# ylsung/vl-merging

Measured on AMD Instinct MI355X. Metric: VL samples/sec (fwd+bwd) base_vl 384^2 at 1/2/4/8 GPUs; merge GB/s vs HBM peak, higher is better.
Workload: dtype bf16

## Files before the change

### include/vlm_hip.h

```cpp
#ifndef VLM_HIP_H
#define VLM_HIP_H
#include <stddef.h>
#include <stdint.h>

#ifdef __cplusplus
extern "C" {
#endif

#define VLM_OK 0
#define VLM_ERR_ARG (-1)
#define VLM_ERR_LAUNCH (-2)
#define VLM_ERR_WORKSPACE (-3)
#define VLM_ERR_UNSUPPORTED (-4)

#define VLM_ABI_VERSION 10
int vlm_abi_version(void);
int vlm_device_cus(void);
int vlm_set_cu_budget(int cus);
int vlm_debug_occupy(int workgroups, int threads, int lds_bytes, int microseconds, void* stream);

#define VLM_MERGE_LERP 0
#define VLM_MERGE_TASKVEC 1
#define VLM_MERGE_MEAN 2
#define VLM_MERGE_MAX_SRC 4
// ... 70 lines not shown

int vlm_gemm_bf16(int ta, int tb, int M, int N, int K, const void* A, int lda, const void* B, int ldb, void* C,
                  int ldc, int c_is_f32, const vlm_epilogue_t* epi, void* stream);
#define VLM_GEMM_MAX_GROUPS 4
typedef struct {
  int32_t row0, rows;
  const void* B;
  int32_t ldb;
  int32_t reserved;
  const float* bias;
  float* col_sum;
  float* col_sum_ws;
} vlm_gemm_group_t;
int vlm_gemm_bf16_grouped(int n_groups, const vlm_gemm_group_t* groups, int N, int K, const void* A, int lda, void* C,
                          int ldc, int c_is_f32, const vlm_epilogue_t* epi, void* stream);
typedef struct {
  int32_t row0, rows;
  float* C;
  int32_t accumulate;
  int32_t reserved;
} vlm_wgrad_group_t;
int vlm_gemm_wgrad_grouped(int n_groups, const vlm_wgrad_group_t* groups, int M, int N, const void* A, int lda,
                           const void* B, int ldb, int ldc, float* splitk_ws, uint64_t splitk_ws_bytes, void* stream);
int vlm_gemm_set_big_tile_mode(int mode);

int vlm_layernorm_fwd(const float* x, int ldx, int M, int D, const float* gamma, const float* beta, float eps,
                      void* y, int ldy, int y_is_f32, float* stats, void* stream);
#define VLM_ROW_WS_BYTES(D) ((size_t)1536 * 2 * (size_t)(D) * sizeof(float))
int vlm_layernorm_bwd(const void* dy, int lddy, int dy_is_f32, const float* x, int ldx, const float* stats,
                      const float* gamma, int M, int D, const float* dres, int lddres, float* dx, int lddx,
                      float* dgamma, float* dbeta, float* workspace, size_t workspace_bytes, int* deferred_blocks,
                      void* stream);
typedef struct {
  const void* y;
  int32_t ldy;
  const float* gamma;
  const float* row_scale;
  void* dy;
  int32_t lddy;
  float* dgamma;
  float* dbias;
  float* workspace;
  size_t workspace_bytes;
} vlm_layerscale_t;
int vlm_layernorm_bwd_scale(const void* dy, int lddy, int dy_is_f32, const float* x, int ldx, const float* stats,
                            const float* gamma, int M, int D, const float* dres, int lddres, float* dx, int lddx,
// ... 156 lines not shown
```

### vl-merging_amd/_lib.py

```python
import ctypes
import os

_HERE = os.path.dirname(os.path.abspath(__file__))
LIB_PATH = os.environ.get("VLM_LIB_PATH") or os.path.join(_HERE, "lib", "libvlm_hip.so")
_lib = None

c_void_p = ctypes.c_void_p
c_int = ctypes.c_int
c_float = ctypes.c_float
c_size_t = ctypes.c_size_t
c_u64 = ctypes.c_uint64

MERGE_LERP, MERGE_TASKVEC, MERGE_MEAN = 0, 1, 2
MERGE_MAX_SRC = 4


class MergeJob(ctypes.Structure):
    _fields_ = [
        ("dst", c_void_p),
        ("base", c_void_p),
        ("src", c_void_p * MERGE_MAX_SRC),
        ("ratio", c_float * MERGE_MAX_SRC),
        ("n_src", ctypes.c_int32),
        ("mode", ctypes.c_int32),
# ... 30 lines not shown
                ("row_step", ctypes.c_int32), ("count", ctypes.c_int32)]


class Epilogue(ctypes.Structure):
    _fields_ = [
        ("bias", c_void_p), ("col_scale", c_void_p), ("row_scale", c_void_p), ("residual", c_void_p),
        ("ld_res", ctypes.c_int64), ("aux", c_void_p), ("ld_aux", ctypes.c_int64), ("act", ctypes.c_int32),
        ("alpha", c_float), ("accumulate", ctypes.c_int32), ("reserved", ctypes.c_int32), ("col_sum", c_void_p),
        ("col_sum_ws", c_void_p), ("splitk_ws", c_void_p), ("splitk_ws_bytes", ctypes.c_uint64),
    ]


GEMM_MAX_GROUPS = 4


class GemmGroup(ctypes.Structure):
    _fields_ = [("row0", ctypes.c_int32), ("rows", ctypes.c_int32), ("B", c_void_p), ("ldb", ctypes.c_int32),
                ("reserved", ctypes.c_int32), ("bias", c_void_p), ("col_sum", c_void_p), ("col_sum_ws", c_void_p)]


class WgradGroup(ctypes.Structure):
    _fields_ = [("row0", ctypes.c_int32), ("rows", ctypes.c_int32), ("C", c_void_p), ("accumulate", ctypes.c_int32),
                ("reserved", ctypes.c_int32)]


class FoldJob(ctypes.Structure):
    _fields_ = [("partials", c_void_p), ("nblocks", ctypes.c_int32), ("D", ctypes.c_int32), ("out0", c_void_p),
                ("out1", c_void_p)]


class LayerScale(ctypes.Structure):
    _fields_ = [("y", c_void_p), ("ldy", ctypes.c_int32), ("gamma", c_void_p), ("row_scale", c_void_p), ("dy", c_void_p),
                ("lddy", ctypes.c_int32), ("dgamma", c_void_p), ("dbias", c_void_p), ("workspace", c_void_p),
                ("workspace_bytes", c_size_t)]


class AttnColsum(ctypes.Structure):
    _fields_ = [("dq", c_void_p * 2), ("dv", c_void_p * 2)]


ACT_NONE, ACT_GELU, ACT_GELU_BWD, ACT_GELU_DERIV, ACT_MUL_AUX = 0, 1, 2, 3, 4
ATTN_JOINT, ATTN_SEPARATE = 0, 1


class AttnDesc(ctypes.Structure):
    _fields_ = [
# ... 22 lines not shown


_ERR = {-1: "VLM_ERR_ARG", -2: "VLM_ERR_LAUNCH", -3: "VLM_ERR_WORKSPACE", -4: "VLM_ERR_UNSUPPORTED"}

SIGNATURES = {
    "vlm_abi_version": (c_int, []),
    "vlm_device_cus": (c_int, []),
    "vlm_set_cu_budget": (c_int, [c_int]),
    "vlm_debug_occupy": (c_int, [c_int, c_int, c_int, c_int, c_void_p]),
    "vlm_layerscale_fold": (c_int, [ctypes.POINTER(LayerScaleJob), c_int, c_void_p]),
    "vlm_layerscale_finish": (c_int, [ctypes.POINTER(LayerScaleJob), c_int, c_void_p]),
    "vlm_merge_plan_bytes": (c_size_t, [c_int, c_u64]),
    "vlm_merge_plan_upload": (c_int, [ctypes.POINTER(MergeJob), c_int, c_void_p, c_size_t, c_void_p]),
    "vlm_merge_run": (c_int, [c_void_p, c_void_p]),
    "vlm_ties_plan_bytes": (c_size_t, [c_int, c_u64]),
    "vlm_ties_plan_upload": (c_int, [ctypes.POINTER(TiesJob), c_int, c_void_p, c_size_t, c_void_p]),
    "vlm_ties_run": (c_int, [c_void_p, c_void_p]),
    "vlm_gemm_bf16": (c_int, [c_int, c_int, c_int, c_int, c_int, c_void_p, c_int, c_void_p, c_int, c_void_p, c_int,
                              c_int, ctypes.POINTER(Epilogue), c_void_p]),
    "vlm_gemm_bf16_grouped": (c_int, [c_int, ctypes.POINTER(GemmGroup), c_int, c_int, c_void_p, c_int, c_void_p, c_int, c_int,
                                      ctypes.POINTER(Epilogue), c_void_p]),
    "vlm_gemm_wgrad_grouped": (c_int, [c_int, ctypes.POINTER(WgradGroup), c_int, c_int, c_void_p, c_int, c_void_p, c_int, c_int,
                                       c_void_p, c_u64, c_void_p]),
    "vlm_attention_fwd": (c_int, [ctypes.POINTER(AttnDesc), c_void_p, c_int, c_void_p, c_void_p]),
    "vlm_attention_bwd_ws_floats": (c_size_t, [ctypes.POINTER(AttnDesc), c_int]),
    "vlm_attention_bwd": (c_int, [ctypes.POINTER(AttnDesc), c_void_p, c_int, c_void_p, c_int, c_void_p, c_void_p, c_size_t,
                                  c_void_p, c_int, c_void_p, c_void_p, c_void_p]),
    "vlm_layernorm_fwd": (c_int, [c_void_p, c_int, c_int, c_int, c_void_p, c_void_p, c_float, c_void_p, c_int, c_int,
                                  c_void_p, c_void_p]),
    "vlm_layernorm_bwd": (c_int, [c_void_p, c_int, c_int, c_void_p, c_int, c_void_p, c_void_p, c_int, c_int, c_void_p,
                                  c_int, c_void_p, c_int, c_void_p, c_void_p, c_void_p, c_size_t,
                                  ctypes.POINTER(c_int), c_void_p]),
    "vlm_layernorm_bwd_scale": (c_int, [c_void_p, c_int, c_int, c_void_p, c_int, c_void_p, c_void_p, c_int, c_int, c_void_p,
                                        c_int, c_void_p, c_int, c_void_p, c_void_p, c_void_p, c_size_t,
                                        ctypes.POINTER(LayerScale), ctypes.POINTER(c_int), c_void_p]),
    "vlm_layerscale_bwd": (c_int, [c_void_p, c_int, c_void_p, c_int, c_void_p, c_void_p, c_int, c_int, c_void_p, c_int,
                                   c_void_p, c_void_p, c_void_p, c_size_t, ctypes.POINTER(c_int), c_void_p]),
    "vlm_colreduce_batch": (c_int, [ctypes.POINTER(FoldJob), c_int, c_void_p]),
    "vlm_gemm_set_big_tile_mode": (c_int, [c_int]),
    "vlm_colsum_bf16": (c_int, [c_void_p, c_int, c_int, c_int, c_void_p, c_void_p]),
    "vlm_adamw_step": (c_int, [c_void_p, c_void_p, c_void_p, c_void_p, c_void_p, c_u64, c_float, c_float, c_float,
                               c_float, c_float, c_float, c_float, c_int, c_void_p]),
    "vlm_accumulate_f32_f64": (c_int, [c_void_p, c_void_p, c_u64, c_void_p]),
    "vlm_gram_f64": (c_int, [c_void_p, c_int, c_int, c_int, c_int, c_void_p, c_void_p]),
    "vlm_gemm_f64": (c_int, [c_int, c_int, c_int, c_int, c_int, ctypes.c_double, c_void_p, c_int, c_int, c_void_p, c_int,
                             ctypes.c_double, c_void_p, c_int, c_void_p]),
# ... 85 lines not shown
```

### vl-merging_amd/csrc/gemm.hip

```cpp
#include "vlm_common.h"
#include "vlm_diag.h"
#include <atomic>

#define GEMM_BM 128
#define GEMM_BN 128
#define GEMM_BK 64
#define GEMM_THREADS 256
#define GEMM_TILE_BYTES (GEMM_BM * GEMM_BK * 2)

typedef __attribute__((address_space(3))) s16x4 lds_s16x4;

__device__ __forceinline__ float gelu_cdf(float x, float& ez2) {
  const float t = __builtin_amdgcn_rcpf(fmaf(0.3275911f * 0.70710678118654752440f, fabsf(x), 1.0f));
  ez2 = __builtin_amdgcn_exp2f((x * x) * (-0.5f * 1.4426950408889634f));
  float poly = fmaf(t, 0.5f * 1.061405429f, 0.5f * -1.453152027f);
  poly = fmaf(t, poly, 0.5f * 1.421413741f);
  poly = fmaf(t, poly, 0.5f * -0.284496736f);
  poly = fmaf(t, poly, 0.5f * 0.254829592f);
  const float e = fmaf(-(poly * t), ez2, 0.5f);
  return 0.5f + copysignf(e, x);
}
__device__ __forceinline__ float gelu_erf(float x) {
  float ez2;
  return x * gelu_cdf(x, ez2);
}
// ... 885 lines not shown
#define BIG_TAIL_STEPS()                                                               \
  BIG_STEP(kt + 0, 0, 1, 1, fa0, fb0, fa1, fb1, ra0, rb0, sA0, sB0, sA1, sB1)          \
  BIG_STEP(kt + 1, 0, 1, 1, fa1, fb1, fa0, fb0, ra1, rb1, sA1, sB1, sA0, sB0)          \
  BIG_STEP(kt + 2, 0, 0, 1, fa0, fb0, fa1, fb1, ra0, rb0, sA0, sB0, sA1, sB1)          \
  BIG_STEP(kt + 3, 0, 0, 0, fa1, fb1, fa0, fb0, ra1, rb1, sA1, sB1, sA0, sB0)
  if constexpr (DEEP) {
    BIG_TAIL_STEPS()
    GEMM_STAMP(2)
    big_epilogue_t<OUT_F32, RES, AUX> ep(p, wl, mw0, nw0, lane);
    float* ws_row = (p.epi.col_sum_ws && mw0 + 128 <= (uint32_t)p.M) ? p.epi.col_sum_ws + ((size_t)(tm_ws * 2 + wm) * 2) * p.N : nullptr;
    BIG_EPILOGUE_LOOP_DEEP(AHEAD)
    ep.finish(lane, ws_row);
  } else {
    EPIL_SETUP()
    BIG_TAIL_STEPS()
    GEMM_STAMP(2)
    float* ws_row = (p.epi.col_sum_ws && mw0 + 128 <= (uint32_t)p.M) ? p.epi.col_sum_ws + ((size_t)(tm_ws * 2 + wm) * 2) * p.N : nullptr;
    BIG_EPILOGUE_LOOP()
    ep.finish(lane, ws_row);
  }
  GEMM_STAMP_END()
}

template <bool GROUPED = false>
__global__ __launch_bounds__(GEMM_THREADS, 1) void vlm_gemm_bigT_kernel(const gemm_params_t p) {
  __shared__ __attribute__((aligned(1024))) unsigned char sA0[BIG_OP_BYTES], sA1[BIG_OP_BYTES], sB0[BIG_OP_BYTES], sB1[BIG_OP_BYTES];
  __shared__ __attribute__((aligned(16))) unsigned char epl[4 * EPIL_WAVE_BYTES];
  const int tid = threadIdx.x;
  const int lane = tid & 63;
  const int wave = __builtin_amdgcn_readfirstlane(tid >> 6);
  const int wm = wave >> 1, wn = wave & 1;
  const uint32_t ntile = p.tiles_m * p.tiles_n;
  const uint32_t q8 = gridDim.x >> 3, r8 = gridDim.x & 7, xcd = blockIdx.x & 7;
  uint32_t item = (xcd < r8 ? xcd * (q8 + 1) : r8 * (q8 + 1) + (xcd - r8) * q8) + (blockIdx.x >> 3);
  uint32_t k_base = 0, k_end = (uint32_t)p.K, slice0 = 0;
  int nk = p.ksteps_per_split;
  if constexpr (GROUPED) {
    int g = 0;
#pragma unroll
    for (int i = 1; i < VLM_GEMM_MAX_GROUPS; ++i)
      if (i < p.n_groups && item >= (uint32_t)p.grpT[i].item0) g = i;
    const gemmT_group_t G = p.grpT[g];
    item -= (uint32_t)G.item0;
    k_base = (uint32_t)G.row0;
    k_end = (uint32_t)G.row_end;
    nk = G.kps;
    slice0 = (uint32_t)G.slice0;
  }
  const uint32_t split = item / ntile, tile = item - split * ntile;
  const uint32_t tm = tile / p.tiles_n, tn = tile - tm * p.tiles_n;
  const uint32_t m0 = tm * BIG_BM, n0 = tn * BIG_BN;
  const uint32_t k_first = k_base + split * (uint32_t)nk * BIG_BK;
  const __amdgpu_buffer_rsrc_t ra =
      __builtin_amdgcn_make_buffer_rsrc(const_cast<void*>(p.A), 0, (int)((uint64_t)k_end * p.lda * 2), 0x00020000);
  const __amdgpu_buffer_rsrc_t rb =
      __builtin_amdgcn_make_buffer_rsrc(const_cast<void*>(p.B), 0, (int)((uint64_t)k_end * p.ldb * 2), 0x00020000);

  uint32_t offa[4], offb[4], wr_off[4];
#pragma unroll
  for (int u = 0; u < 4; ++u) {
    const uint32_t row = 2 * (wave + 4 * u) + (lane >> 5), c16 = lane & 31;
    offa[u] = ((k_first + row) * (uint32_t)p.lda + m0 + c16 * 8) * 2;
    offb[u] = ((k_first + row) * (uint32_t)p.ldb + n0 + c16 * 8) * 2;
    wr_off[u] = row * 512 + (((c16 >> 1) ^ ((row & 3) | (((row >> 3) & 1) << 2))) << 5) + (c16 & 1) * 16;
  }
  uint32_t rda[8], rdb[8];
  {
    const uint32_t g = lane >> 4, q = (lane & 15) >> 2, pp = lane & 3, sw = q | ((g & 1) << 2);
#pragma unroll
    for (int i = 0; i < 8; ++i) {
      rda[i] = (8 * g + q) * 512 + wm * 256 + ((i ^ sw) << 5) + 8 * pp;
      rdb[i] = (8 * g + q) * 512 + wn * 256 + ((i ^ sw) << 5) + 8 * pp;
    }
  }
  f32x4 acc00[4][4], acc01[4][4], acc10[4][4], acc11[4][4];
#pragma unroll
  for (int i = 0; i < 4; ++i)
#pragma unroll
    for (int j = 0; j < 4; ++j) {
      acc00[i][j] = (f32x4){0.f, 0.f, 0.f, 0.f};
      acc01[i][j] = (f32x4){0.f, 0.f, 0.f, 0.f};
      acc10[i][j] = (f32x4){0.f, 0.f, 0.f, 0.f};
      acc11[i][j] = (f32x4){0.f, 0.f, 0.f, 0.f};
    }
  const uint32_t stepa = BIG_BK * (uint32_t)p.lda * 2, stepb = BIG_BK * (uint32_t)p.ldb * 2;
  bf16x8 fa0[8], fb0[8], fa1[8], fb1[8];
  u32x4 ra0[4], rb0[4], ra1[4], rb1[4];
#define BIGT_TR(PTR) __builtin_amdgcn_ds_read_tr16_b64_v4i16((lds_s16x4*)(PTR))
#define BIGT_READ(FA, FB, SA, SB)                                                                    \
  _Pragma("unroll") for (int i = 0; i < 8; ++i) {                                                    \
    const s16x4 al = BIGT_TR((SA) + rda[i]), ah = BIGT_TR((SA) + rda[i] + 4 * 512);                  \
    const s16x4 bl = BIGT_TR((SB) + rdb[i]), bh = BIGT_TR((SB) + rdb[i] + 4 * 512);                  \
    FA[i] = __builtin_bit_cast(bf16x8, (s16x8){al[0], al[1], al[2], al[3], ah[0], ah[1], ah[2], ah[3]}); \
    FB[i] = __builtin_bit_cast(bf16x8, (s16x8){bl[0], bl[1], bl[2], bl[3], bh[0], bh[1], bh[2], bh[3]}); \
  }
#define BIGT_GLOAD(RA_, RB_, S)                                                                      \
  _Pragma("unroll") for (int u = 0; u < 4; ++u) {                                                    \
    RA_[u] = __builtin_amdgcn_raw_buffer_load_b128(ra, offa[u], (S) * stepa, 0);                     \
    RB_[u] = __builtin_amdgcn_raw_buffer_load_b128(rb, offb[u], (S) * stepb, 0);                     \
  }
#define BIGT_LWRITE(RA_, RB_, SA, SB)                                                                \
  _Pragma("unroll") for (int u = 0; u < 4; ++u) {                                                    \
    *reinterpret_cast<u32x4*>((SA) + wr_off[u]) = RA_[u];                                            \
    *reinterpret_cast<u32x4*>((SB) + wr_off[u]) = RB_[u];                                            \
  }
#define BIGT_STEP(K, GL, WR, RD, FCA, FCB, FNA, FNB, RSA, RSB, BUFA_W, BUFB_W, BUFA_R, BUFB_R)      \
  {                                                                                      \
    if (RD) {                                                                            \
// ... 17 lines not shown
    }                                                                                    \
    __builtin_amdgcn_sched_barrier(0);                                                   \
  }
  BIGT_GLOAD(ra0, rb0, 0)
  BIGT_GLOAD(ra1, rb1, 1)
  BIGT_LWRITE(ra0, rb0, sA0, sB0)
  BIGT_GLOAD(ra0, rb0, 2)
  BIGT_LWRITE(ra1, rb1, sA1, sB1)
  BIGT_GLOAD(ra1, rb1, 3)
  asm volatile("s_waitcnt lgkmcnt(0)" ::: "memory");
  __builtin_amdgcn_s_barrier();
  BIGT_READ(fa0, fb0, sA0, sB0)
  int kt = 0;
  for (; kt < nk - 4; kt += 2) {
    BIGT_STEP(kt + 0, 1, 1, 1, fa0, fb0, fa1, fb1, ra0, rb0, sA0, sB0, sA1, sB1)
    BIGT_STEP(kt + 1, 1, 1, 1, fa1, fb1, fa0, fb0, ra1, rb1, sA1, sB1, sA0, sB0)
  }
  BIGT_STEP(kt + 0, 0, 1, 1, fa0, fb0, fa1, fb1, ra0, rb0, sA0, sB0, sA1, sB1)
  BIGT_STEP(kt + 1, 0, 1, 1, fa1, fb1, fa0, fb0, ra1, rb1, sA1, sB1, sA0, sB0)
  BIGT_STEP(kt + 2, 0, 0, 1, fa0, fb0, fa1, fb1, ra0, rb0, sA0, sB0, sA1, sB1)
  BIGT_STEP(kt + 3, 0, 0, 0, fa1, fb1, fa0, fb0, ra1, rb1, sA1, sB1, sA0, sB0)

  gemm_params_t pl = p;
  pl.C = reinterpret_cast<float*>(p.C) + (size_t)(slice0 + split) * p.M * p.N;
  pl.ldc = p.N;
  const uint32_t mw0 = m0 + wm * 128, nw0 = n0 + wn * 128;
  unsigned char* const wl = epl + wave * EPIL_WAVE_BYTES;
  big_epilogue_t<true, false, 0, 128, 0, true> ep(pl, wl, mw0, nw0, lane);
  epil_in_t inA, inB;
  ep.load_inputs(inA, 0);
  BIG_EPILOGUE_LOOP()
}

__global__ __launch_bounds__(256) void splitk_reduce_kernel(const float* __restrict__ ws, int splits, int M, int N, float* __restrict__ C,
                                                            int ldc, int accumulate) {
  const size_t i = (size_t)blockIdx.x * 256 + threadIdx.x, per = (size_t)M * N / 4;
  if (i >= per) return;
  const size_t e = i * 4, m = e / N, n = e - m * N;
  f32x4 t = accumulate ? *reinterpret_cast<const f32x4*>(C + m * ldc + n) : (f32x4){0.f, 0.f, 0.f, 0.f};
  for (int s = 0; s < splits; ++s) t += *reinterpret_cast<const f32x4*>(ws + (size_t)s * M * N + e);
  *reinterpret_cast<f32x4*>(C + m * ldc + n) = t;
}

struct splitk_groups_t {
  float* C[VLM_GEMM_MAX_GROUPS];
  int slice0[VLM_GEMM_MAX_GROUPS], splits[VLM_GEMM_MAX_GROUPS], accumulate[VLM_GEMM_MAX_GROUPS];
};
__global__ __launch_bounds__(256) void splitk_reduce_grouped_kernel(const float* __restrict__ ws, const splitk_groups_t g, int M, int N, int ldc) {
  const size_t i = (size_t)blockIdx.x * 256 + threadIdx.x, per = (size_t)M * N / 4;
  if (i >= per) return;
  const int gi = blockIdx.y;
  float* const C = g.C[gi];
  const size_t e = i * 4, m = e / N, n = e - m * N;
  f32x4 t = g.accumulate[gi] ? *reinterpret_cast<const f32x4*>(C + m * ldc + n) : (f32x4){0.f, 0.f, 0.f, 0.f};
// ... 296 lines not shown
      VLM_CHECK_LAUNCH();
      const size_t per = (size_t)M * N / 4;
      hipLaunchKernelGGL(splitk_reduce_grouped_kernel, dim3((unsigned)((per + 255) / 256), p.n_groups), dim3(256), 0, s,
                         reinterpret_cast<const float*>(splitk_ws), rg, M, N, ldc);
      VLM_CHECK_LAUNCH();
      return VLM_OK;
    }
  }
  for (int g = 0; g < n_groups; ++g) {
    const vlm_wgrad_group_t& G = groups[g];
    if (G.rows == 0) continue;
    vlm_epilogue_t e{};
    e.alpha = 1.0f;
    e.accumulate = G.accumulate;
    e.splitk_ws = splitk_ws;
    e.splitk_ws_bytes = splitk_ws_bytes;
    const size_t r0 = (size_t)G.row0;
    const int rc = vlm_gemm_bf16(1, 1, M, N, G.rows, reinterpret_cast<const unsigned char*>(A) + r0 * lda * 2, lda,
                                 reinterpret_cast<const unsigned char*>(B) + r0 * ldb * 2, ldb, G.C, ldc, 1, &e, stream);
    if (rc) return rc;
  }
  return VLM_OK;
}
```

### vl-merging_amd/engine.py

```python
import itertools
import math
import os
import weakref
from typing import List, Optional

import torch

from . import _lib as L
from . import ops

BF16, F32 = torch.bfloat16, torch.float32
ALIGN = 64


def _touch_hook(p):
    p._vlm_flat.touched.add(p._vlm_name)


def touch(*params):
    for p in params:
        if p is not None:
            f = getattr(p, "_vlm_flat", None)
            if f is not None:
                f.touched.add(p._vlm_name)
# ... 208 lines not shown
        return False


def wT16(p):
    s = getattr(p, "_vlm_bf16_t", None)
    if s is None:
        raise L.VlmError("weight has no transposed bf16 shadow: call model.setup_engine() on a CUDA model first")
    return s


def _gemm_rows(a, groups, out, *, act=L.ACT_NONE, aux=None, col_scale=None, row_scale=None, residual=None, col_sum_fold=None):
    if len(groups) > 1:
        return ops.gemm_grouped(a, groups, out, act=act, aux=aux, col_scale=col_scale, row_scale=row_scale,
                                residual=residual, col_sum_fold=col_sum_fold)
    (r0, r1, w, bias, col_sum), = groups

    def rows(t):
        return t[r0:r1] if t is not None else None

    return ops.gemm(a[r0:r1], w, out[r0:r1], bias=bias, act=act, aux=rows(aux), col_scale=col_scale,
                    row_scale=rows(row_scale), residual=rows(residual), col_sum=col_sum, col_sum_fold=col_sum_fold)


def _wgrad_rows(dy, x, groups):
    if len(groups) > 1:
        return ops.gemm_wgrad_grouped(dy, x, groups)
    (r0, r1, dw), = groups
    return ops.gemm(dy[r0:r1], x[r0:r1], dw, ta=True, tb=True, accumulate=True)


def w16(p):
    s = getattr(p, "_vlm_bf16", None)
    if s is None:
        raise L.VlmError("parameter has no bf16 shadow: call model.setup_engine() on a CUDA model first")
    return s


class RelPos:

    def __init__(self, bias_t, index16, index16_t, holder, cache_tag=None, cache=None):
        self.bias_t = bias_t
        self.index = index16
        self.index_t = index16_t
        self.holder = holder
        self._dense = {}
        self.cache_tag = cache_tag
        self.cache = cache

    def dense_for(self, seq, mode):
        key = (seq.n0, seq.n1, seq.pos1, mode)
        d = self._dense.get(key)
# ... 345 lines not shown
            flat = plan.ranges[0][2].projw._vlm_flat
            _arm_layerscale_finish(flat)
        wg = (lambda w: w._vlm_raw) if folded else (lambda w: w.grad)
        touch(g1, g2)
        for _, _, e in plan.ranges:
            _touch_expert(e)
        dy2 = torch.empty(M, D, device=dev, dtype=BF16)
        dy1 = torch.empty(M, D, device=dev, dtype=BF16)
        dh = torch.empty(M, Fdim, device=dev, dtype=BF16)
        dln = torch.empty(M, D, device=dev, dtype=BF16)
        dx1 = torch.empty(M, D, device=dev, dtype=F32)
        fold = ops.FoldBatch(dev, D)
        rg = plan.ranges
        do = torch.empty(M, D, device=dev, dtype=BF16)
        for r0, r1, e in rg:
            rr = slice(r0, r1)
            if folded:
                ops.layerscale_bwd(dx2[rr], None, None, rs2[rr] if rs2 is not None else None, dy2[rr], None, _rb(e.fc2b), fold=fold)
            else:
                ops.layerscale_bwd(dx2[rr], y2[rr], g2, rs2[rr] if rs2 is not None else None, dy2[rr], g2.grad, e.fc2b.grad,
                                   fold=fold)
        _gemm_rows(dy2, [(r0, r1, wT16(e.fc2w), None, e.fc1b.grad) for r0, r1, e in rg], dh, act=L.ACT_MUL_AUX, aux=h,
                   col_sum_fold=fold)
        with _Side(dy2, a, dh, ln2):
            _wgrad_rows(dy2, a, [(r0, r1, wg(e.fc2w)) for r0, r1, e in rg])
            _wgrad_rows(dh, ln2, [(r0, r1, e.fc1w.grad) for r0, r1, e in rg])
        _gemm_rows(dh, [(r0, r1, wT16(e.fc1w), None, None) for r0, r1, e in rg], dln)
        for r0, r1, e in rg:
            rr = slice(r0, r1)
            _ln2_bwd_scale1(dln[rr], x1[rr], st2[rr], e, dx1[rr], dx2[rr], y1[rr] if y1 is not None else None, g1,
                            rs1[rr] if rs1 is not None else None, dy1[rr], fold)
        _gemm_rows(dy1, [(r0, r1, wT16(e.projw), None, None) for r0, r1, e in rg], do)
        with _Side(dy1, o):
            _wgrad_rows(dy1, o, [(r0, r1, wg(e.projw)) for r0, r1, e in rg])
        dqkv = torch.empty(M, 3 * D, device=dev, dtype=BF16)
        dln1 = torch.empty(M, D, device=dev, dtype=BF16)
        rp = pc.relpos
        qb_grads, vb_grads, fused_qv = _segment_bias_grads(rg, pc.seq)
        ops.attention_bwd(qkv, o, do, lse, dqkv, pc.seq, H, bias_t=bias_t, head_row0=plan.layer * H,
                          rel_index=rp.index if rp is not None else None,
                          rel_index_t=rp.index_t if rp is not None else None, keep0=pc.keep0, keep1=pc.keep1,
                          mode=plan.mode, dbias_t=rp.holder.get("dbias_t") if rp is not None else None,
                          dq_colsum=qb_grads, dv_colsum=vb_grads,
                          bias_dense=rp.dense_for(pc.seq, plan.mode) if rp is not None else None)
        dx = torch.empty(M, D, device=dev, dtype=F32)
        for r0, r1, e in rg:
            if e.qb is not None and not fused_qv:
                ops.colsum(dqkv[r0:r1, :D], e.qb.grad)
                ops.colsum(dqkv[r0:r1, 2 * D:], e.vb.grad)
        with _Side(dqkv, ln1):
            _wgrad_rows(dqkv, ln1, [(r0, r1, e.qkvw.grad) for r0, r1, e in rg])
        _gemm_rows(dqkv, [(r0, r1, wT16(e.qkvw), None, None) for r0, r1, e in rg], dln1)
        for r0, r1, e in rg:
            rr = slice(r0, r1)
            ops.layernorm_bwd(dln1[rr], x[rr], st1[rr], e.n1w, dx[rr], dres=dx1[rr], dgamma=e.n1w.grad, dbeta=e.n1b.grad,
                              fold=fold)
        fold.flush()
        if folded:
            flat.ls_pending.add(plan.layer)
        if ctx.hook is not None:
            ctx.hook(plan.layer)
        dbias = None
        if bias_t is not None and ctx.needs_input_grad[1] and rp is not None and not rp.holder.get("routed"):
            rp.holder["routed"] = True
            dbias = _zero_scalar(dev).expand_as(bias_t)
        return dx, dbias, None, None, None, None


def run_block(x, plan: BlockPlan, pc: PassCtx, training: bool, hook=None):
    bias_t = pc.relpos.bias_t if pc.relpos is not None else None
    return _BlockFn.apply(x, bias_t, plan, pc, training, hook)


class _LinearFn(torch.autograd.Function):
# ... 472 lines not shown
```

### vl-merging_amd/ops.py

```python
import ctypes

import torch

from . import _lib as L

BF16 = torch.bfloat16
F32 = torch.float32


def _ld(t):
    if t.dim() != 2 or t.stride(1) != 1:
        raise L.VlmError("expected a 2-D tensor with unit inner stride, got shape %s strides %s"
                         % (tuple(t.shape), t.stride()))
    return t.stride(0) if t.shape[0] > 1 else max(t.stride(0), t.shape[1])


def gemm(a, b, out, ta=False, tb=False, *, bias=None, act=L.ACT_NONE, aux=None, col_scale=None, row_scale=None,
         residual=None, alpha=1.0, accumulate=False, col_sum=None, col_sum_fold=None):
    L.require_cuda(a, b, out, bias, aux, col_scale, row_scale, residual, col_sum)
    if a.dtype != BF16 or b.dtype != BF16:
        raise L.VlmError("gemm operands must be bfloat16")
    M, N = out.shape
    K = a.shape[0] if ta else a.shape[1]
    if (a.shape[1] if ta else a.shape[0]) != M:
# ... 95 lines not shown

def gemm_wgrad_grouped(dy, x, groups, accumulate=True):
    L.require_cuda(dy, x)
    if dy.dtype != BF16 or x.dtype != BF16 or dy.shape[0] != x.shape[0]:
        raise L.VlmError("gemm_wgrad_grouped: bf16 dy [tokens, M] and x [tokens, N]")
    M, N = dy.shape[1], x.shape[1]
    arr = (L.WgradGroup * len(groups))()
    prev, ldc = 0, None
    for g, (r0, r1, dW) in zip(arr, groups):
        L.require_cuda(dW)
        if dW.dtype != F32 or tuple(dW.shape) != (M, N) or r0 < prev or r1 < r0 or r1 > dy.shape[0]:
            raise L.VlmError("gemm_wgrad_grouped: group (%d, %d) gradient %s for M=%d N=%d" % (r0, r1, tuple(dW.shape), M, N))
        if ldc is not None and _ld(dW) != ldc:
            raise L.VlmError("gemm_wgrad_grouped: the groups' gradients must share one leading dimension")
        ldc = _ld(dW)
        prev = r1
        g.row0, g.rows, g.C, g.accumulate = r0, r1 - r0, dW.data_ptr(), int(bool(accumulate))
    ws = _splitk_workspace(dy.device)
    rc = L.get_lib().vlm_gemm_wgrad_grouped(len(groups), arr, M, N, L.ptr(dy), _ld(dy), L.ptr(x), _ld(x), ldc, L.ptr(ws),
                                            ws.numel() * 4, L.stream_ptr())
    L.check(rc, "vlm_gemm_wgrad_grouped")


_SPLITK_WS = {}
SPLITK_WS_BYTES = 96 << 20


def _splitk_workspace(device):
    key = (device.index, torch.cuda.current_stream().cuda_stream)
    ws = _SPLITK_WS.get(key)
    if ws is None:
        ws = _SPLITK_WS[key] = torch.empty(SPLITK_WS_BYTES // 4, device=device, dtype=F32)
    return ws


def layernorm_fwd(x, gamma, beta, eps, out, stats=None):
    L.require_cuda(x, gamma, beta, out, stats)
    M, D = x.shape
    rc = L.get_lib().vlm_layernorm_fwd(L.ptr(x), _ld(x), M, D, L.ptr(gamma), L.ptr(beta), eps, L.ptr(out), _ld(out),
                                       int(out.dtype == F32), L.ptr(stats), L.stream_ptr())
    L.check(rc, "vlm_layernorm_fwd")
    return out


_ROW_WS = {}


def _row_workspace(device, D, slot=0):
# ... 739 lines not shown
```

Before: 335.9.

## Batch all block weight-gradient GEMMs into one load-balanced multi-job kernel

Replaces the per-layer weight-gradient GEMM calls (fc2, fc1, proj, qkv) with a single multi-job launch. A host-side planner splits every output tile's K range into segments, balances the work across the CUs, writes partials to a workspace and reduces them with a second kernel. The plan table is cached per shape. The aim is to remove tail underutilisation and launch overhead from several small split-K GEMMs. In exchange it adds a reduce pass, more workspace traffic and a larger split-K workspace, and the wgrads now run later in the backward pass on the side stream.

```diff
diff --git a/include/vlm_hip.h b/include/vlm_hip.h
--- a/include/vlm_hip.h
+++ b/include/vlm_hip.h
@@ -116,6 +116,22 @@
 } vlm_wgrad_group_t;
 int vlm_gemm_wgrad_grouped(int n_groups, const vlm_wgrad_group_t* groups, int M, int N, const void* A, int lda,
                            const void* B, int ldb, int ldc, float* splitk_ws, uint64_t splitk_ws_bytes, void* stream);
+#define VLM_WGRAD_MAX_JOBS 8
+typedef struct {
+  const void* A;
+  const void* B;
+  float* C;
+  int32_t lda, ldb, ldc;
+  int32_t M, N;
+  int32_t row0, rows;
+  int32_t accumulate;
+} vlm_wgrad_job_t;
+int vlm_gemm_wgrad_multi(int n_jobs, const vlm_wgrad_job_t* jobs, float* splitk_ws, uint64_t splitk_ws_bytes, void* stream);
+typedef struct {
+  int32_t job, tile_m, tile_n, k0, k1, ws_slot;
+} vlm_wgrad_seg_t;
+int vlm_wgrad_multi_plan(int n_jobs, const int32_t* M, const int32_t* N, const int32_t* rows, int cus, int32_t* wg_first, int wg_cap,
+                         vlm_wgrad_seg_t* segs, int seg_cap, int* n_wgs);
 int vlm_gemm_set_big_tile_mode(int mode);
 
 int vlm_layernorm_fwd(const float* x, int ldx, int M, int D, const float* gamma, const float* beta, float eps,
diff --git a/vl-merging_amd/_lib.py b/vl-merging_amd/_lib.py
--- a/vl-merging_amd/_lib.py
+++ b/vl-merging_amd/_lib.py
@@ -76,6 +76,20 @@
 class WgradGroup(ctypes.Structure):
     _fields_ = [("row0", ctypes.c_int32), ("rows", ctypes.c_int32), ("C", c_void_p), ("accumulate", ctypes.c_int32),
                 ("reserved", ctypes.c_int32)]
+
+
+WGRAD_MAX_JOBS = 8
+
+
+class WgradJob(ctypes.Structure):
+    _fields_ = [("A", c_void_p), ("B", c_void_p), ("C", c_void_p), ("lda", ctypes.c_int32), ("ldb", ctypes.c_int32),
+                ("ldc", ctypes.c_int32), ("M", ctypes.c_int32), ("N", ctypes.c_int32), ("row0", ctypes.c_int32),
+                ("rows", ctypes.c_int32), ("accumulate", ctypes.c_int32)]
+
+
+class WgradSeg(ctypes.Structure):
+    _fields_ = [("job", ctypes.c_int32), ("tile_m", ctypes.c_int32), ("tile_n", ctypes.c_int32), ("k0", ctypes.c_int32),
+                ("k1", ctypes.c_int32), ("ws_slot", ctypes.c_int32)]
 
 
 class FoldJob(ctypes.Structure):
@@ -144,6 +158,10 @@
                                       ctypes.POINTER(Epilogue), c_void_p]),
     "vlm_gemm_wgrad_grouped": (c_int, [c_int, ctypes.POINTER(WgradGroup), c_int, c_int, c_void_p, c_int, c_void_p, c_int, c_int,
                                        c_void_p, c_u64, c_void_p]),
+    "vlm_gemm_wgrad_multi": (c_int, [c_int, ctypes.POINTER(WgradJob), c_void_p, c_u64, c_void_p]),
+    "vlm_wgrad_multi_plan": (c_int, [c_int, ctypes.POINTER(ctypes.c_int32), ctypes.POINTER(ctypes.c_int32),
+                                     ctypes.POINTER(ctypes.c_int32), c_int, ctypes.POINTER(ctypes.c_int32), c_int,
+                                     ctypes.POINTER(WgradSeg), c_int, ctypes.POINTER(c_int)]),
     "vlm_attention_fwd": (c_int, [ctypes.POINTER(AttnDesc), c_void_p, c_int, c_void_p, c_void_p]),
     "vlm_attention_bwd_ws_floats": (c_size_t, [ctypes.POINTER(AttnDesc), c_int]),
     "vlm_attention_bwd": (c_int, [ctypes.POINTER(AttnDesc), c_void_p, c_int, c_void_p, c_int, c_void_p, c_void_p, c_size_t,
diff --git a/vl-merging_amd/csrc/gemm.hip b/vl-merging_amd/csrc/gemm.hip
--- a/vl-merging_amd/csrc/gemm.hip
+++ b/vl-merging_amd/csrc/gemm.hip
@@ -1,6 +1,10 @@
 #include "vlm_common.h"
 #include "vlm_diag.h"
+#include <algorithm>
 #include <atomic>
+#include <map>
+#include <mutex>
+#include <vector>
 
 #define GEMM_BM 128
 #define GEMM_BN 128
@@ -932,46 +936,26 @@
   GEMM_STAMP_END()
 }
 
-template <bool GROUPED = false>
-__global__ __launch_bounds__(GEMM_THREADS, 1) void vlm_gemm_bigT_kernel(const gemm_params_t p) {
+__device__ __forceinline__ void gemm_bigT_tile(const gemm_params_t& p, float* C, const int ldc, const void* A, const void* B, const uint32_t lda,
+                                               const uint32_t ldb, const uint32_t k_end, const uint32_t k_first, const int nk,
+                                               const uint32_t m0, const uint32_t n0, const uint32_t mw0, const uint32_t nw0) {
   __shared__ __attribute__((aligned(1024))) unsigned char sA0[BIG_OP_BYTES], sA1[BIG_OP_BYTES], sB0[BIG_OP_BYTES], sB1[BIG_OP_BYTES];
   __shared__ __attribute__((aligned(16))) unsigned char epl[4 * EPIL_WAVE_BYTES];
   const int tid = threadIdx.x;
   const int lane = tid & 63;
   const int wave = __builtin_amdgcn_readfirstlane(tid >> 6);
   const int wm = wave >> 1, wn = wave & 1;
-  const uint32_t ntile = p.tiles_m * p.tiles_n;
-  const uint32_t q8 = gridDim.x >> 3, r8 = gridDim.x & 7, xcd = blockIdx.x & 7;
-  uint32_t item = (xcd < r8 ? xcd * (q8 + 1) : r8 * (q8 + 1) + (xcd - r8) * q8) + (blockIdx.x >> 3);
-  uint32_t k_base = 0, k_end = (uint32_t)p.K, slice0 = 0;
-  int nk = p.ksteps_per_split;
-  if constexpr (GROUPED) {
-    int g = 0;
-#pragma unroll
-    for (int i = 1; i < VLM_GEMM_MAX_GROUPS; ++i)
-      if (i < p.n_groups && item >= (uint32_t)p.grpT[i].item0) g = i;
-    const gemmT_group_t G = p.grpT[g];
-    item -= (uint32_t)G.item0;
-    k_base = (uint32_t)G.row0;
-    k_end = (uint32_t)G.row_end;
-    nk = G.kps;
-    slice0 = (uint32_t)G.slice0;
-  }
-  const uint32_t split = item / ntile, tile = item - split * ntile;
-  const uint32_t tm = tile / p.tiles_n, tn = tile - tm * p.tiles_n;
-  const uint32_t m0 = tm * BIG_BM, n0 = tn * BIG_BN;
-  const uint32_t k_first = k_base + split * (uint32_t)nk * BIG_BK;
   const __amdgpu_buffer_rsrc_t ra =
-      __builtin_amdgcn_make_buffer_rsrc(const_cast<void*>(p.A), 0, (int)((uint64_t)k_end * p.lda * 2), 0x00020000);
+      __builtin_amdgcn_make_buffer_rsrc(const_cast<void*>(A), 0, (int)((uint64_t)k_end * lda * 2), 0x00020000);
   const __amdgpu_buffer_rsrc_t rb =
-      __builtin_amdgcn_make_buffer_rsrc(const_cast<void*>(p.B), 0, (int)((uint64_t)k_end * p.ldb * 2), 0x00020000);
+      __builtin_amdgcn_make_buffer_rsrc(const_cast<void*>(B), 0, (int)((uint64_t)k_end * ldb * 2), 0x00020000);
 
   uint32_t offa[4], offb[4], wr_off[4];
 #pragma unroll
   for (int u = 0; u < 4; ++u) {
     const uint32_t row = 2 * (wave + 4 * u) + (lane >> 5), c16 = lane & 31;
-    offa[u] = ((k_first + row) * (uint32_t)p.lda + m0 + c16 * 8) * 2;
-    offb[u] = ((k_first + row) * (uint32_t)p.ldb + n0 + c16 * 8) * 2;
+    offa[u] = ((k_first + row) * lda + m0 + c16 * 8) * 2;
+    offb[u] = ((k_first + row) * ldb + n0 + c16 * 8) * 2;
     wr_off[u] = row * 512 + (((c16 >> 1) ^ ((row & 3) | (((row >> 3) & 1) << 2))) << 5) + (c16 & 1) * 16;
   }
   uint32_t rda[8], rdb[8];
@@ -993,7 +977,7 @@
       acc10[i][j] = (f32x4){0.f, 0.f, 0.f, 0.f};
       acc11[i][j] = (f32x4){0.f, 0.f, 0.f, 0.f};
     }
-  const uint32_t stepa = BIG_BK * (uint32_t)p.lda * 2, stepb = BIG_BK * (uint32_t)p.ldb * 2;
+  const uint32_t stepa = BIG_BK * lda * 2, stepb = BIG_BK * ldb * 2;
   bf16x8 fa0[8], fb0[8], fa1[8], fb1[8];
   u32x4 ra0[4], rb0[4], ra1[4], rb1[4];
 #define BIGT_TR(PTR) __builtin_amdgcn_ds_read_tr16_b64_v4i16((lds_s16x4*)(PTR))
@@ -1057,14 +1041,103 @@
   BIGT_STEP(kt + 3, 0, 0, 0, fa1, fb1, fa0, fb0, ra1, rb1, sA1, sB1, sA0, sB0)
 
   gemm_params_t pl = p;
-  pl.C = reinterpret_cast<float*>(p.C) + (size_t)(slice0 + split) * p.M * p.N;
-  pl.ldc = p.N;
-  const uint32_t mw0 = m0 + wm * 128, nw0 = n0 + wn * 128;
+  pl.C = C;
+  pl.ldc = ldc;
   unsigned char* const wl = epl + wave * EPIL_WAVE_BYTES;
   big_epilogue_t<true, false, 0, 128, 0, true> ep(pl, wl, mw0, nw0, lane);
   epil_in_t inA, inB;
   ep.load_inputs(inA, 0);
   BIG_EPILOGUE_LOOP()
+}
+
+template <bool GROUPED = false>
+__global__ __launch_bounds__(GEMM_THREADS, 1) void vlm_gemm_bigT_kernel(const gemm_params_t p) {
+  const int wave = __builtin_amdgcn_readfirstlane(threadIdx.x >> 6);
+  const int wm = wave >> 1, wn = wave & 1;
+  const uint32_t ntile = p.tiles_m * p.tiles_n;
+  const uint32_t q8 = gridDim.x >> 3, r8 = gridDim.x & 7, xcd = blockIdx.x & 7;
+  uint32_t item = (xcd < r8 ? xcd * (q8 + 1) : r8 * (q8 + 1) + (xcd - r8) * q8) + (blockIdx.x >> 3);
+  uint32_t k_base = 0, k_end = (uint32_t)p.K, slice0 = 0;
+  int nk = p.ksteps_per_split;
+  if constexpr (GROUPED) {
+    int g = 0;
+#pragma unroll
+    for (int i = 1; i < VLM_GEMM_MAX_GROUPS; ++i)
+      if (i < p.n_groups && item >= (uint32_t)p.grpT[i].item0) g = i;
+    const gemmT_group_t G = p.grpT[g];
+    item -= (uint32_t)G.item0;
+    k_base = (uint32_t)G.row0;
+    k_end = (uint32_t)G.row_end;
+    nk = G.kps;
+    slice0 = (uint32_t)G.slice0;
+  }
+  const uint32_t split = item / ntile, tile = item - split * ntile;
+  const uint32_t tm = tile / p.tiles_n, tn = tile - tm * p.tiles_n;
+  const uint32_t m0 = tm * BIG_BM, n0 = tn * BIG_BN;
+  const uint32_t k_first = k_base + split * (uint32_t)nk * BIG_BK;
+  gemm_bigT_tile(p, reinterpret_cast<float*>(p.C) + (size_t)(slice0 + split) * p.M * p.N, p.N, p.A, p.B, (uint32_t)p.lda,
+                 (uint32_t)p.ldb, k_end, k_first, nk, m0, n0, m0 + wm * 128, n0 + wn * 128);
+}
+
+struct wgm_job_t {
+  const void* A;
+  const void* B;
+  float* C;
+  int lda, ldb, ldc, row0, row_end, accumulate;
+};
+struct wgm_params_t {
+  const int* wg_first;
+  const int* segs;
+  const int* tiles;
+  float* ws;
+  wgm_job_t job[VLM_WGRAD_MAX_JOBS];
+};
+#define WGM_TILE_FLOATS (BIG_BM * BIG_BN)
+
+#define WGM_JOB_FIELD(J, FIELD, DST)                                     \
+  DST = q.job[0].FIELD;                                                  \
+  _Pragma("unroll") for (int i_ = 1; i_ < VLM_WGRAD_MAX_JOBS; ++i_) if (i_ == (J)) DST = q.job[i_].FIELD;
+
+__global__ __launch_bounds__(GEMM_THREADS, 1) void vlm_wgrad_multi_kernel(const wgm_params_t q) {
+  const int wave = __builtin_amdgcn_readfirstlane(threadIdx.x >> 6);
+  const int wm = wave >> 1, wn = wave & 1;
+  const int s0 = q.wg_first[blockIdx.x], s1 = q.wg_first[blockIdx.x + 1];
+  gemm_params_t pl;
+  pl.epi = vlm_epilogue_t{};
+  pl.epi.alpha = 1.0f;
+  pl.M = BIG_BM;
+  pl.N = BIG_BN;
+  for (int s = s0; s < s1; ++s) {
+    if (s > s0) __syncthreads();
+    int sg[6];
+#pragma unroll
+    for (int i = 0; i < 6; ++i) sg[i] = __builtin_amdgcn_readfirstlane(q.segs[6 * s + i]);
+    const void *A, *B;
+    int lda, ldb, row0, row_end;
+    WGM_JOB_FIELD(sg[0], A, A)
+    WGM_JOB_FIELD(sg[0], B, B)
+    WGM_JOB_FIELD(sg[0], lda, lda)
+    WGM_JOB_FIELD(sg[0], ldb, ldb)
+    WGM_JOB_FIELD(sg[0], row0, row0)
+    WGM_JOB_FIELD(sg[0], row_end, row_end)
+    gemm_bigT_tile(pl, q.ws + (size_t)sg[5] * WGM_TILE_FLOATS, BIG_BN, A, B, (uint32_t)lda, (uint32_t)ldb, (uint32_t)row_end,
+                   (uint32_t)(row0 + sg[3] * BIG_BK), sg[4], (uint32_t)sg[1], (uint32_t)sg[2], wm * 128, wn * 128);
+  }
+}
+
+__global__ __launch_bounds__(256) void wgrad_multi_reduce_kernel(const wgm_params_t q) {
+  const int* t = q.tiles + 5 * blockIdx.y;
+  float* C;
+  int ldc, accumulate;
+  WGM_JOB_FIELD(t[0], C, C)
+  WGM_JOB_FIELD(t[0], ldc, ldc)
+  WGM_JOB_FIELD(t[0], accumulate, accumulate)
+  const uint32_t e = (blockIdx.x * 256 + threadIdx.x) * 4, r = e / BIG_BN, c = e % BIG_BN;
+  float* const dst = C + (size_t)(t[1] + r) * ldc + t[2] + c;
+  f32x4 v = accumulate ? *reinterpret_cast<const f32x4*>(dst) : (f32x4){0.f, 0.f, 0.f, 0.f};
+  const float* src = q.ws + (size_t)t[3] * WGM_TILE_FLOATS + e;
+  for (int i = 0; i < t[4]; ++i) v += *reinterpret_cast<const f32x4*>(src + (size_t)i * WGM_TILE_FLOATS);
+  *reinterpret_cast<f32x4*>(dst) = v;
 }
 
 __global__ __launch_bounds__(256) void splitk_reduce_kernel(const float* __restrict__ ws, int splits, int M, int N, float* __restrict__ C,
@@ -1407,3 +1480,268 @@
   }
   return VLM_OK;
 }
+
+static const int WGM_MIN_UNITS = 8;
+static const int WGM_SEG_COST_UNITS = 10;
+
+struct wgm_plan_t {
+  std::vector<int> wg_first;
+  std::vector<vlm_wgrad_seg_t> segs;
+  std::vector<int> tiles;
+};
+
+static void wgm_plan(int n, const int* Mj, const int* Nj, const int* rows, int cus, wgm_plan_t& P) {
+  struct tile_t { int job, tm, tn, u, ksteps, full, rem; };
+  struct run_t { std::vector<vlm_wgrad_seg_t> segs; };
+  std::vector<tile_t> T;
+  long U = 0;
+  for (int j = 0; j < n; ++j) {
+    if (rows[j] <= 0) continue;
+    const int ks = (rows[j] + BIG_BK - 1) / BIG_BK, u = (ks + 1) / 2;
+    for (int tm = 0; tm < Mj[j] / BIG_BM; ++tm)
+      for (int tn = 0; tn < Nj[j] / BIG_BN; ++tn) { T.push_back(tile_t{j, tm, tn, u, ks, 0, 0}); U += u; }
+  }
+  P.wg_first.assign(1, 0);
+  P.segs.clear();
+  P.tiles.clear();
+  if (T.empty()) return;
+  const int G = (int)std::min<long>(cus, std::max<long>(1, U / WGM_MIN_UNITS));
+  const long L0 = (U + G - 1) / G;
+  auto cut = [&](long L, bool apply, long& n_al, long& R, long& pieces, long& longest) {
+    n_al = R = pieces = 0; longest = 0;
+    for (tile_t& t : T) {
+      int full = (int)(t.u / L), rem = (int)(t.u - full * L);
+      if (full > 0 && rem > 0 && rem < WGM_MIN_UNITS) { longest = std::max<long>(longest, L + rem); rem = 0; }
+      else if (full > 0) longest = std::max<long>(longest, L);
+      n_al += full; R += rem; pieces += rem > 0;
+      if (apply) { t.full = full; t.rem = rem; }
+    }
+  };
+  long bestL = L0;
+  double best = 1e30;
+  for (long L = L0; L <= L0 + L0 / 4 + 1; ++L) {
+    long n_al, R, pieces, longest;
+    cut(L, false, n_al, R, pieces, longest);
+    const long n_lo = G - n_al;
+    if (n_lo < 0 || (R > 0 && n_lo == 0)) continue;
+    const double c_al = n_al ? (double)longest + WGM_SEG_COST_UNITS : 0.0;
+    const double c_lo = R ? (double)R / n_lo + WGM_SEG_COST_UNITS * ((double)pieces / n_lo + 1.0) : 0.0;
+    const double c = std::max(c_al, c_lo);
+    if (c < best) { best = c; bestL = L; }
+  }
+  long n_al, R, pieces, longest;
+  cut(bestL, true, n_al, R, pieces, longest);
+  const long L = bestL;
+  std::vector<run_t> runs;
+  int max_full = 0;
+  for (const tile_t& t : T) max_full = std::max(max_full, t.full);
+  for (int f = 0; f < max_full; ++f)
+    for (size_t i = 0; i < T.size(); ++i) {
+      const tile_t& t = T[i];
+      if (f >= t.full) continue;
+      const long u0 = f * L, u1 = (f == t.full - 1 && t.rem == 0) ? t.u : (f + 1) * L;
+      run_t r;
+      r.segs.push_back(vlm_wgrad_seg_t{(int32_t)i, t.tm, t.tn, (int32_t)(2 * u0), (int32_t)std::min<long>(2 * u1, t.ksteps), 0});
+      runs.push_back(r);
+    }
+  const size_t n_aligned = runs.size();
+  if (R > 0) {
+    long n_lo = std::min<long>(G - n_al, std::max<long>(1, R / WGM_MIN_UNITS));
+    std::vector<long> b(n_lo + 1);
+    for (long w = 0; w <= n_lo; ++w) {
+      long x = w * R / n_lo, t0 = 0;
+      for (const tile_t& t : T) {
+        if (!t.rem) continue;
+        const long t1 = t0 + t.rem;
+        if (x > t0 && x < t1) {
+          if (x - t0 < WGM_MIN_UNITS) x = t0;
+          else if (t1 - x < WGM_MIN_UNITS) x = t1;
+          break;
+        }
+        t0 = t1;
+      }
+      b[w] = x;
+    }
+    for (long w = 0; w < n_lo; ++w) {
+      if (b[w + 1] <= b[w]) continue;
+      run_t r;
+      long t0 = 0;
+      for (size_t i = 0; i < T.size(); ++i) {
+        const tile_t& t = T[i];
+        if (!t.rem) continue;
+        const long t1 = t0 + t.rem, lo = std::max(b[w], t0), hi = std::min(b[w + 1], t1);
+        if (lo < hi) {
+          const long base = (long)t.full * L - t0;
+          r.segs.push_back(vlm_wgrad_seg_t{(int32_t)i, t.tm, t.tn, (int32_t)(2 * (lo + base)),
+                                           (int32_t)std::min<long>(2 * (hi + base), t.ksteps), 0});
+        }
+        t0 = t1;
+      }
+      runs.push_back(r);
+    }
+  }
+  std::vector<int> count(T.size(), 0), slot0(T.size(), 0);
+  for (const run_t& r : runs)
+    for (const vlm_wgrad_seg_t& sgm : r.segs) ++count[sgm.job];
+  for (size_t i = 1; i < T.size(); ++i) slot0[i] = slot0[i - 1] + count[i - 1];
+  for (run_t& r : runs)
+    for (vlm_wgrad_seg_t& sgm : r.segs) {
+      int before = 0;
+      for (const run_t& r2 : runs)
+        for (const vlm_wgrad_seg_t& o : r2.segs) before += (o.job == sgm.job && o.k0 < sgm.k0);
+      sgm.ws_slot = slot0[sgm.job] + before;
+    }
+  for (size_t i = 0; i < T.size(); ++i) {
+    const int v[5] = {T[i].job, T[i].tm * BIG_BM, T[i].tn * BIG_BN, slot0[i], count[i]};
+    P.tiles.insert(P.tiles.end(), v, v + 5);
+  }
+  const size_t W = runs.size();
+  std::vector<int> order(W, -1);
+  std::vector<size_t> used(8, 0), cap(8);
+  for (size_t x = 0; x < 8; ++x) cap[x] = W / 8 + (x < W % 8);
+  std::vector<char> placed(W, 0);
+  for (size_t x = 0; x < 8; ++x)
+    for (size_t r = x * n_aligned / 8; r < (x + 1) * n_aligned / 8 && used[x] < cap[x]; ++r) {
+      order[x + 8 * used[x]++] = (int)r;
+      placed[r] = 1;
+    }
+  size_t x = 0;
+  for (size_t r = 0; r < W; ++r) {
+    if (placed[r]) continue;
+    while (used[x] >= cap[x]) ++x;
+    order[x + 8 * used[x]++] = (int)r;
+  }
+  for (size_t w = 0; w < W; ++w) {
+    for (vlm_wgrad_seg_t sgm : runs[order[w]].segs) {
+      sgm.job = T[sgm.job].job;
+      P.segs.push_back(sgm);
+    }
+    P.wg_first.push_back((int)P.segs.size());
+  }
+}
+
+extern "C" int vlm_wgrad_multi_plan(int n_jobs, const int32_t* M, const int32_t* N, const int32_t* rows, int cus, int32_t* wg_first,
+                                    int wg_cap, vlm_wgrad_seg_t* segs, int seg_cap, int* n_wgs) {
+  if (n_jobs < 0 || n_jobs > VLM_WGRAD_MAX_JOBS || cus < 1 || (n_jobs && (!M || !N || !rows))) return VLM_ERR_ARG;
+  for (int j = 0; j < n_jobs; ++j)
+    if (M[j] <= 0 || N[j] <= 0 || (M[j] % BIG_BM) || (N[j] % BIG_BN) || rows[j] < 0) return VLM_ERR_ARG;
+  wgm_plan_t P;
+  wgm_plan(n_jobs, M, N, rows, cus, P);
+  const int W = (int)P.wg_first.size() - 1;
+  if (n_wgs) *n_wgs = W;
+  if (wg_first) {
+    if (wg_cap < W + 1) return VLM_ERR_WORKSPACE;
+    for (int w = 0; w <= W; ++w) wg_first[w] = P.wg_first[w];
+  }
+  if (segs) {
+    if (seg_cap < (int)P.segs.size()) return VLM_ERR_WORKSPACE;
+    for (size_t i = 0; i < P.segs.size(); ++i) segs[i] = P.segs[i];
+  }
+  return (int)P.segs.size();
+}
+
+struct wgm_table_t {
+  int* dev = nullptr;
+  int n_wgs = 0, n_segs = 0, n_tiles = 0;
+};
+static std::mutex g_wgm_mu;
+static std::map<std::vector<int>, wgm_table_t> g_wgm_tables;
+
+static const wgm_table_t* wgm_table(int n, const int* Mj, const int* Nj, const int* rows, int cus) {
+  int dev = 0;
+  if (hipGetDevice(&dev) != hipSuccess) return nullptr;
+  std::vector<int> key{dev, cus, n};
+  for (int j = 0; j < n; ++j) { key.push_back(Mj[j]); key.push_back(Nj[j]); key.push_back(rows[j]); }
+  std::lock_guard<std::mutex> lock(g_wgm_mu);
+  auto it = g_wgm_tables.find(key);
+  if (it != g_wgm_tables.end()) return &it->second;
+  if (g_wgm_tables.size() >= 256) {
+    for (auto& kv : g_wgm_tables) (void)hipFree(kv.second.dev);
+    g_wgm_tables.clear();
+  }
+  wgm_plan_t P;
+  wgm_plan(n, Mj, Nj, rows, cus, P);
+  wgm_table_t t;
+  t.n_wgs = (int)P.wg_first.size() - 1;
+  t.n_segs = (int)P.segs.size();
+  t.n_tiles = (int)P.tiles.size() / 5;
+  std::vector<int> h(P.wg_first);
+  for (const vlm_wgrad_seg_t& sgm : P.segs) {
+    int nk = sgm.k1 - sgm.k0;
+    nk += nk & 1;
+    const int v[6] = {sgm.job, sgm.tile_m * BIG_BM, sgm.tile_n * BIG_BN, sgm.k0, nk < 4 ? 4 : nk, sgm.ws_slot};
+    h.insert(h.end(), v, v + 6);
+  }
+  h.insert(h.end(), P.tiles.begin(), P.tiles.end());
+  if (hipMalloc(&t.dev, h.size() * sizeof(int)) != hipSuccess) return nullptr;
+  if (hipMemcpy(t.dev, h.data(), h.size() * sizeof(int), hipMemcpyHostToDevice) != hipSuccess) {
+    (void)hipFree(t.dev);
+    return nullptr;
+  }
+  return &(g_wgm_tables[key] = t);
+}
+
+extern "C" int vlm_gemm_wgrad_multi(int n_jobs, const vlm_wgrad_job_t* jobs, float* splitk_ws, uint64_t splitk_ws_bytes, void* stream) {
+  if (n_jobs < 0 || n_jobs > VLM_WGRAD_MAX_JOBS || (n_jobs && !jobs)) return VLM_ERR_ARG;
+  bool multi = gemm_big_mode() > 0 && splitk_ws && ((uintptr_t)splitk_ws & 15) == 0;
+  int live = 0;
+  for (int j = 0; j < n_jobs; ++j) {
+    const vlm_wgrad_job_t& J = jobs[j];
+    if (J.M < 0 || J.N < 0 || J.row0 < 0 || J.rows < 0 || !J.C) return VLM_ERR_ARG;
+    if (J.M == 0 || J.N == 0 || J.rows == 0) continue;
+    if (!J.A || !J.B || (J.lda & 7) || (J.ldb & 7) || ((uintptr_t)J.A & 15) || ((uintptr_t)J.B & 15) || J.lda < J.M || J.ldb < J.N ||
+        J.ldc < J.N)
+      return VLM_ERR_ARG;
+    ++live;
+    const uint64_t row_end = (uint64_t)J.row0 + J.rows;
+    if ((J.M % BIG_BM) || (J.N % BIG_BN) || (J.ldc & 3) || ((uintptr_t)J.C & 15) || row_end * J.lda * 2 >= (1ull << 31) ||
+        row_end * J.ldb * 2 >= (1ull << 31))
+      multi = false;
+  }
+  hipStream_t s = (hipStream_t)stream;
+  for (int j = 0; j < n_jobs; ++j) {
+    const vlm_wgrad_job_t& J = jobs[j];
+    if (J.rows == 0 && J.M > 0 && J.N > 0 && !J.accumulate &&
+        hipMemset2DAsync(J.C, (size_t)J.ldc * 4, 0, (size_t)J.N * 4, J.M, s) != hipSuccess)
+      return VLM_ERR_LAUNCH;
+  }
+  if (live == 0) return VLM_OK;
+  if (multi) {
+    wgm_params_t q{};
+    int Mj[VLM_WGRAD_MAX_JOBS], Nj[VLM_WGRAD_MAX_JOBS], rows[VLM_WGRAD_MAX_JOBS], n = 0;
+    for (int j = 0; j < n_jobs; ++j) {
+      const vlm_wgrad_job_t& J = jobs[j];
+      if (J.M == 0 || J.N == 0 || J.rows == 0) continue;
+      Mj[n] = J.M; Nj[n] = J.N; rows[n] = J.rows;
+      q.job[n] = wgm_job_t{J.A, J.B, J.C, J.lda, J.ldb, J.ldc, J.row0, J.row0 + J.rows, J.accumulate};
+      ++n;
+    }
+    const wgm_table_t* t = wgm_table(n, Mj, Nj, rows, plan_cus());
+    if (!t) return VLM_ERR_LAUNCH;
+    if ((uint64_t)t->n_segs * WGM_TILE_FLOATS * 4 <= splitk_ws_bytes) {
+      q.wg_first = t->dev;
+      q.segs = t->dev + t->n_wgs + 1;
+      q.tiles = q.segs + 6 * (size_t)t->n_segs;
+      q.ws = splitk_ws;
+      hipLaunchKernelGGL(vlm_wgrad_multi_kernel, dim3(t->n_wgs), dim3(GEMM_THREADS), 0, s, q);
+      VLM_CHECK_LAUNCH();
+      hipLaunchKernelGGL(wgrad_multi_reduce_kernel, dim3(WGM_TILE_FLOATS / 4 / 256, t->n_tiles), dim3(256), 0, s, q);
+      VLM_CHECK_LAUNCH();
+      return VLM_OK;
+    }
+  }
+  for (int j = 0; j < n_jobs; ++j) {
+    const vlm_wgrad_job_t& J = jobs[j];
+    if (J.M == 0 || J.N == 0 || J.rows == 0) continue;
+    vlm_epilogue_t e{};
+    e.alpha = 1.0f;
+    e.accumulate = J.accumulate;
+    e.splitk_ws = splitk_ws;
+    e.splitk_ws_bytes = splitk_ws_bytes;
+    const size_t r0 = (size_t)J.row0;
+    const int rc = vlm_gemm_bf16(1, 1, J.M, J.N, J.rows, reinterpret_cast<const unsigned char*>(J.A) + r0 * J.lda * 2, J.lda,
+                                 reinterpret_cast<const unsigned char*>(J.B) + r0 * J.ldb * 2, J.ldb, J.C, J.ldc, 1, &e, stream);
+    if (rc) return rc;
+  }
+  return VLM_OK;
+}
diff --git a/vl-merging_amd/engine.py b/vl-merging_amd/engine.py
--- a/vl-merging_amd/engine.py
+++ b/vl-merging_amd/engine.py
@@ -254,11 +254,9 @@
                     row_scale=rows(row_scale), residual=rows(residual), col_sum=col_sum, col_sum_fold=col_sum_fold)
 
 
-def _wgrad_rows(dy, x, groups):
-    if len(groups) > 1:
-        return ops.gemm_wgrad_grouped(dy, x, groups)
-    (r0, r1, dw), = groups
-    return ops.gemm(dy[r0:r1], x[r0:r1], dw, ta=True, tb=True, accumulate=True)
+def _wgrad_block(jobs):
+    for i in range(0, len(jobs), L.WGRAD_MAX_JOBS):
+        ops.gemm_wgrad_multi(jobs[i:i + L.WGRAD_MAX_JOBS])
 
 
 def w16(p):
@@ -650,17 +648,15 @@
                                    fold=fold)
         _gemm_rows(dy2, [(r0, r1, wT16(e.fc2w), None, e.fc1b.grad) for r0, r1, e in rg], dh, act=L.ACT_MUL_AUX, aux=h,
                    col_sum_fold=fold)
-        with _Side(dy2, a, dh, ln2):
-            _wgrad_rows(dy2, a, [(r0, r1, wg(e.fc2w)) for r0, r1, e in rg])
-            _wgrad_rows(dh, ln2, [(r0, r1, e.fc1w.grad) for r0, r1, e in rg])
+        wjobs = [(dy2, a, r0, r1, wg(e.fc2w), True) for r0, r1, e in rg]
+        wjobs += [(dh, ln2, r0, r1, e.fc1w.grad, True) for r0, r1, e in rg]
         _gemm_rows(dh, [(r0, r1, wT16(e.fc1w), None, None) for r0, r1, e in rg], dln)
         for r0, r1, e in rg:
             rr = slice(r0, r1)
             _ln2_bwd_scale1(dln[rr], x1[rr], st2[rr], e, dx1[rr], dx2[rr], y1[rr] if y1 is not None else None, g1,
                             rs1[rr] if rs1 is not None else None, dy1[rr], fold)
         _gemm_rows(dy1, [(r0, r1, wT16(e.projw), None, None) for r0, r1, e in rg], do)
-        with _Side(dy1, o):
-            _wgrad_rows(dy1, o, [(r0, r1, wg(e.projw)) for r0, r1, e in rg])
+        wjobs += [(dy1, o, r0, r1, wg(e.projw), True) for r0, r1, e in rg]
         dqkv = torch.empty(M, 3 * D, device=dev, dtype=BF16)
         dln1 = torch.empty(M, D, device=dev, dtype=BF16)
         rp = pc.relpos
@@ -676,8 +672,9 @@
             if e.qb is not None and not fused_qv:
                 ops.colsum(dqkv[r0:r1, :D], e.qb.grad)
                 ops.colsum(dqkv[r0:r1, 2 * D:], e.vb.grad)
-        with _Side(dqkv, ln1):
-            _wgrad_rows(dqkv, ln1, [(r0, r1, e.qkvw.grad) for r0, r1, e in rg])
+        wjobs += [(dqkv, ln1, r0, r1, e.qkvw.grad, True) for r0, r1, e in rg]
+        with _Side(dy2, a, dh, ln2, dy1, o, dqkv, ln1):
+            _wgrad_block(wjobs)
         _gemm_rows(dqkv, [(r0, r1, wT16(e.qkvw), None, None) for r0, r1, e in rg], dln1)
         for r0, r1, e in rg:
             rr = slice(r0, r1)
diff --git a/vl-merging_amd/ops.py b/vl-merging_amd/ops.py
--- a/vl-merging_amd/ops.py
+++ b/vl-merging_amd/ops.py
@@ -141,8 +141,43 @@
     L.check(rc, "vlm_gemm_wgrad_grouped")
 
 
+def gemm_wgrad_multi(jobs):
+    if len(jobs) > L.WGRAD_MAX_JOBS:
+        raise L.VlmError("gemm_wgrad_multi: at most %d jobs" % L.WGRAD_MAX_JOBS)
+    if not jobs:
+        return
+    arr = (L.WgradJob * len(jobs))()
+    for g, (dy, x, r0, r1, dW, accumulate) in zip(arr, jobs):
+        L.require_cuda(dy, x, dW)
+        if dy.dtype != BF16 or x.dtype != BF16 or dW.dtype != F32 or dy.shape[0] != x.shape[0]:
+            raise L.VlmError("gemm_wgrad_multi: bf16 dy [tokens, M] and x [tokens, N], f32 dW")
+        if tuple(dW.shape) != (dy.shape[1], x.shape[1]) or r0 < 0 or r1 < r0 or r1 > dy.shape[0]:
+            raise L.VlmError("gemm_wgrad_multi: rows (%d, %d) gradient %s for dy %s x %s"
+                             % (r0, r1, tuple(dW.shape), tuple(dy.shape), tuple(x.shape)))
+        g.A, g.B, g.C = dy.data_ptr(), x.data_ptr(), dW.data_ptr()
+        g.lda, g.ldb, g.ldc = _ld(dy), _ld(x), _ld(dW)
+        g.M, g.N, g.row0, g.rows, g.accumulate = dy.shape[1], x.shape[1], r0, r1 - r0, int(bool(accumulate))
+    ws = _splitk_workspace(jobs[0][0].device)
+    rc = L.get_lib().vlm_gemm_wgrad_multi(len(jobs), arr, L.ptr(ws), ws.numel() * 4, L.stream_ptr())
+    L.check(rc, "vlm_gemm_wgrad_multi")
+
+
+def wgrad_multi_plan(shapes, rows, cus):
+    n = len(shapes)
+    i32 = ctypes.c_int32 * max(n, 1)
+    Ms, Ns, Rs = i32(*[m for m, _ in shapes]), i32(*[k for _, k in shapes]), i32(*rows)
+    lib = L.get_lib()
+    n_wgs = ctypes.c_int(0)
+    n_segs = lib.vlm_wgrad_multi_plan(n, Ms, Ns, Rs, cus, None, 0, None, 0, ctypes.byref(n_wgs))
+    L.check(min(n_segs, 0), "vlm_wgrad_multi_plan")
+    first = (ctypes.c_int32 * (n_wgs.value + 1))()
+    segs = (L.WgradSeg * max(n_segs, 1))()
+    L.check(min(lib.vlm_wgrad_multi_plan(n, Ms, Ns, Rs, cus, first, n_wgs.value + 1, segs, n_segs, None), 0), "vlm_wgrad_multi_plan")
+    return list(first), [(g.job, g.tile_m, g.tile_n, g.k0, g.k1, g.ws_slot) for g in segs[:n_segs]]
+
+
 _SPLITK_WS = {}
-SPLITK_WS_BYTES = 96 << 20
+SPLITK_WS_BYTES = (256 + 216) * 256 * 1024
 
 
 def _splitk_workspace(device):
```

Result: no change. 335.7 (median of 3 runs) (-0.1%).
